# ComputationalRobotics/XM-code

Measured on AMD Instinct MI355X. Metric: BM iters/sec (tCG Hessian-vector iterations per second; ms_per_step = wall-clock-to-KKT of one staircase solve), higher is better.
Workload: dtype f64

## Files before the change

### xm-code_amd/csrc/xm_common.h

```cpp
#pragma once

#include <hip/hip_runtime.h>

#include <algorithm>
#include <cstdint>
#include <cstdio>
#include <stdexcept>
#include <string>
#include <vector>

namespace xm {

struct Error : std::runtime_error {
    int code;
    Error(int c, const std::string &m) : std::runtime_error(m), code(c) {}
};

#define XM_HIP_CHECK(expr)                                                                            \
    do {                                                                                              \
        hipError_t _e = (expr);                                                                       \
        if (_e != hipSuccess)                                                                         \
            throw ::xm::Error(-3, std::string("HIP error: ") + hipGetErrorString(_e) + " at " +       \
                                      __FILE__ + ":" + std::to_string(__LINE__) + " (" #expr ")");    \
    } while (0)
// ... 156 lines not shown
    const double *ps_cur;
    double *ps_next;
    double *vR, *vs, *HvR, *Hvs, *rR;
    const double *rs_cur;
    double *rs_next;
    double *Wloc, *Wpad;
    PointPtrs cur, cand;
    const double *partsA;
    double *partsM;
    int nM;
    double delta_bar, gradtol;
    int max_outer;
    double *trace;
    int trace_cap;
    const int *stop_req;
    unsigned long long *hprog;
    unsigned int run;
    int slot, grp;
};
void launch_outer_step(int o, int polar, const OuterStepArgs &A, int grid, hipStream_t st);

struct TcgParity {
    TcgScal *scal_cur, *scal_next;
    double *ps_cur, *ps_next, *rs_cur, *rs_next;
    size_t chunk, b_off;
    double *pcur;
    double *parts;
    double *Bout;
    double *partsB_out;
};

struct TcgInitArgs {
    int nloc;
    const double *rgR, *rgs, *R, *s;
    double *rR, *rs, *pR, *ps, *vR, *vs, *HvR, *Hvs;
    double *Wloc, *Wpad;
    TcgScal *scal0;
    double rr, delta;
    unsigned long long *hstat;
    int seq;
    const SpecCtl *spec;
};
struct CgStepArgs {
    int nloc;
    TcgParity v;
    int nA, nB, world;
    const double *HpR, *Hps, *R, *s;
    double *pR, *vR, *vs, *HvR, *Hvs, *rR;
    double *Wloc, *Wpad;
    unsigned long long *hstat;
    int64_t mat;
    double *Afull, *Wfull;
    int grouping;
    PeerXchg xchg;
};

void launch_qw_dense(int o, int epi, const double *Q, int64_t ld, const double *W, double alpha, const CamArgs &a,
                     hipStream_t st);
void launch_qw_bsr3(int o, int epi, const int64_t *rowptr, const int32_t *colidx, const double *blocks, const double *W,
                    double alpha, const CamArgs &a, hipStream_t st, int64_t nb = 0, const int4 *rowinfo = nullptr);
int64_t sell_resident_bytes(int64_t stream, int64_t other);
void bsr_build_rowinfo(const int64_t *rowptr_host, int nloc, std::vector<int4> &out);
int qw_grid(int nloc);
void launch_qw_dense_split(int o, int epi, const double *Q, int64_t ld, const double *W, double alpha, const CamArgs &a, hipStream_t st);
int qw_dense_tile_cols();
int qw_dense_split_k(int nloc, int64_t ld);
int bsr_grid(int nloc);
void qw_bench_nt(int nt);
void symv_bench_k(int k, int kf);
int symv_trace_slots();
struct SymvPlan { int K, Kf, ysplit, nchunks, gx, gy; };
void symv_plan_get(int nloc, int64_t ld, int out[4]);
struct SymvWork {
    int nloc = 0, o = 0;
    int64_t ld = 0;
    SymvPlan plan{};
    DevBuf<double> prow, pcol;
    void ensure(int nloc, int64_t ld, int o);
    void release();
    explicit operator bool() const { return pcol.p != nullptr; }
};
void launch_qw_sym_traced(int o, const double *Q, int64_t ld, const double *W, const CamArgs &a, SymvWork &work, unsigned long long *trace, hipStream_t st);
void launch_qw_sym(int o, int epi, const double *Q, int64_t ld, const double *W, double alpha, const CamArgs &a, SymvWork &work, hipStream_t st,
                   int rev = 0);
void launch_asym(const double *Q, int64_t ld, int64_t m, double *out, int grid, hipStream_t st);
void launch_dense_to_f32(const double *src, float *dst, int64_t rows, int64_t ld, unsigned int *bad, hipStream_t st);
void launch_qw_dense_f32(int o, int epi, const float *Qf, const double *Qd, int64_t ld, const double *W, double alpha, const CamArgs &a, hipStream_t st);
void launch_qw_sym_f32(int o, int epi, const float *Qf, const double *Qd, int64_t ld, const double *W, double alpha, const CamArgs &a, SymvWork &work,
                       hipStream_t st, int rev = 0);

void launch_symhash(const double *Q, int64_t ld, int64_t row0, int64_t nrows, int64_t m, unsigned long long *out, int grid, hipStream_t st);

void launch_transpose_pad(const double *src_colmajor, int64_t lds, int64_t rows, int64_t cols, double *dst, int64_t ldd,
                          hipStream_t st);
void launch_dense_from_bsr(const int64_t *rowptr, const int32_t *colidx, const double *blocks, int64_t nloc, int64_t cam0,
                           double *dst, int64_t ldd, hipStream_t st);

int flat_grid(int64_t elems);
void launch_scale_rows(int o, int nloc, const double *R, const double *s, double *Wloc, hipStream_t st);
void launch_tcg_init(int o, const TcgInitArgs &a, hipStream_t st);
void launch_cg_step(int o, const CgStepArgs &a, hipStream_t st);
struct OuterArgs { double loss, delta, delta_bar, gradtol; int shrink_count, last_iter; };
void launch_outer_finalize(const double *partsA, int nA_loc, int world, const double *partsM, int nM, const TcgScal *scal, double *hres,
                           unsigned long long seq, int grouping, hipStream_t st, const OuterArgs *oa = nullptr, SpecCtl *spec_out = nullptr);
void launch_retract(int o, int nloc, int cam0, const double *R, const double *s, const double *D, const double *ds, double t,
                    double *Rout, double *sout, double *Wloc, hipStream_t st, int polar = 0);
int retract_grid(int nloc);
void launch_retract_model(int o, int nloc, int cam0, const double *R, const double *s, const double *vR, const double *vs, double *Rout, double *sout,
                          double *Wloc, double *Wpad, const double *HvR, const double *Hvs, const double *rgR, const double *rgs, double *parts,
                          hipStream_t st, int polar);
void launch_cert_prepare(int o, int nloc, int cam0, double lam, const double *QsR, const double *R, const double *s,
                         double *Lam, double *dz, double *parts, hipStream_t st);
void launch_recover_gram(int64_t n, int r, const double *R, const double *s, double *parts, int grid, hipStream_t st);
void launch_recover_project(int64_t n, int r, const double *R, const double *s, const double *V, double *rot, double *scale, int *negcount,
                            hipStream_t st, int variant = 0);
void launch_negate(double *x, int64_t len, hipStream_t st);
int dots_multi_segments(int64_t len);
void launch_dots_multi(const double *V, int64_t ldv, int m, const double *w, int64_t len, double *c, double *scratch, hipStream_t st);
void launch_sub_vc(double *w, const double *V, int64_t ldv, const double *c, int m, int64_t len, hipStream_t st);
void launch_scale_copy(double *dst, const double *src, double a, int64_t len, hipStream_t st);
void launch_copy_words(void *dst, const void *src, size_t bytes, hipStream_t st);
void launch_lz_alpha(const double *c1j, const double *c2j, double *alpha_j, hipStream_t st);
void launch_dots_multi_parts(const double *V, int64_t ldv, int m, const double *w, int64_t len, double *scratch, hipStream_t st);
bool lz_fused_ok(int m);
void launch_sub_vc_fin(double *w, const double *V, int64_t ldv, const double *parts, int m, int64_t len, double *c_out, const double *c_prev,
                       double *alpha_j, hipStream_t st);
void launch_lz_next_fin(double *dst, const double *w, const double *parts, double *beta_j, int64_t len, hipStream_t st);
void launch_lz_next(double *dst, const double *w, const double *ww, double *beta_j, int64_t len, hipStream_t st);
void launch_gemv_n(double *y, const double *V, int64_t ldv, const double *c, int m, int64_t len, hipStream_t st);


void launch_edge_locate(int64_t ne, const int32_t *ei, const int32_t *ej, int cam0, int nloc, const int64_t *rowptr, const int32_t *colidx,
                        int64_t *pos_ij, int64_t *pos_ji, int64_t *pos_d, hipStream_t st);
void launch_edge_write(bool dense, int64_t ne, const int32_t *ei, const int32_t *ej, const double *M, const double *w, int cam0, int nloc,
                       const int64_t *inc_ptr, const int32_t *inc_edge, const int64_t *pos_ij, const int64_t *pos_ji, const int64_t *pos_d,
                       double *blocks, double *Q, int64_t ld, hipStream_t st);
void launch_edge_residual(int64_t ne, const int32_t *ei, const int32_t *ej, const double *M, const double *Y, int o, int OP, double *res,
                          hipStream_t st);

void launch_xm2_error(int64_t n, const double *w, const double *res, double *err, hipStream_t st);
void launch_radix_hist(int64_t n, const double *x, int shift, unsigned long long prefix, unsigned int *hist, hipStream_t st);
void launch_xm2_filter(int64_t n, const double *err, const double *w, double thr, double *wout, unsigned int *removed, hipStream_t st);

#define XM_DISPATCH_O(o, CALL)                                                         \
    switch (o) {                                                                       \
        case 1: { constexpr int O_ = 1; CALL; } break;                                 \
        case 3: { constexpr int O_ = 3; CALL; } break;                                 \
        case 4: { constexpr int O_ = 4; CALL; } break;                                 \
        case 5: { constexpr int O_ = 5; CALL; } break;                                 \
        case 6: { constexpr int O_ = 6; CALL; } break;                                 \
        case 7: { constexpr int O_ = 7; CALL; } break;                                 \
        case 8: { constexpr int O_ = 8; CALL; } break;                                 \
        case 9: { constexpr int O_ = 9; CALL; } break;                                 \
        case 10: { constexpr int O_ = 10; CALL; } break;                               \
        default: throw Error(-2, "rank o must be 1 or 3..10, got " + std::to_string(o)); \
    }

inline void check_launch(const char *what) {
    hipError_t e = hipGetLastError();
    if (e != hipSuccess) throw Error(-3, std::string("kernel launch failed (") + what + "): " + hipGetErrorString(e));
}

}
```

### xm-code_amd/csrc/xm_kernels.hip

```cpp
#include <algorithm>
#include <cmath>
#include <cstdlib>
#include <cstring>
#include <type_traits>

#include "xm_common.h"
#include "xm_device.h"
#include "xm_symv_step.h"

namespace xm {

__device__ __forceinline__ double2 nt_load16(const double2 *p) {
    typedef double d2v __attribute__((ext_vector_type(2)));
    const d2v v = __builtin_nontemporal_load(reinterpret_cast<const d2v *>(p));
    return make_double2(v.x, v.y);
}

template <int O, int EPI, int NSUB, bool SPLIT = false>
__global__ __launch_bounds__(256) void qw_dense_kernel(const double *__restrict__ Q, int64_t ld,
                                                        const double *__restrict__ W, double alpha, CamArgs a) {
    constexpr int OP = pitch_of(O);
    int role = EPI;
    constexpr int TILE = NSUB * 128;
    constexpr int TILE2 = TILE * OP / 2;
// ... 2068 lines not shown
        hipLaunchKernelGGL((qw_dense_kernel<1, EPI_CERT, 2>), dim3(qw_grid(a.nloc)), dim3(256), 0, st, Q, ld, W, alpha, ac);
    } else {
        XM_DISPATCH_O(o, (qw_dense_epi<O_, kQwNsub>(epi, Q, ld, W, alpha, a, st)));
    }
    check_launch("qw_dense");
}

static int64_t symv_live_groups(int64_t nsteps, int64_t nstrips, int64_t k) {
    int64_t live = 0;
    for (int64_t s = 0; s < nstrips; ++s) live += (std::min<int64_t>(nsteps, (s * kSvStrip + kSvStrip + 5) / 6) + 4 * k - 1) / (4 * k);
    return live;
}
int symv_k(int nloc, int64_t ld) {
    const int64_t nsteps = (nloc + 1) / 2, nstrips = (ld + kSvStrip - 1) / kSvStrip;
    int64_t total = 0;
    for (int64_t s = 0; s < nstrips; ++s) total += std::min<int64_t>(nsteps, (s * kSvStrip + kSvStrip + 5) / 6);
    int64_t k = (int64_t)(std::sqrt((double)total) / 18.0 + 0.5);
    k = std::min<int64_t>(64, std::max<int64_t>(2, k));
    if (symv_live_groups(nsteps, nstrips, k) <= 1100) {
        int64_t ks = 4;
        while (symv_live_groups(nsteps, nstrips, ks) > 504) ++ks;
        k = ks;
    }
    return (int)k;
}
static int g_symv_k = 0, g_symv_kf = 0;
void symv_bench_k(int k, int kf) { g_symv_k = k; g_symv_kf = kf; }
static SymvPlan symv_plan(int nloc, int64_t ld) {
    SymvPlan p;
    p.K = g_symv_k > 0 ? g_symv_k : symv_k(nloc, ld);
    const int nsteps = (nloc + 1) / 2, nstrips = (int)((ld + kSvStrip - 1) / kSvStrip);
    p.gy = (nstrips + 1) / 2;
    if (g_symv_k > 0 && g_symv_kf > 0) {
        p.Kf = std::min(g_symv_kf, p.K);
        p.ysplit = (int)(0.75 * p.gy);
    } else if (p.K >= 8 && symv_live_groups(nsteps, nstrips, p.K) > 1100) {
        p.Kf = p.K / 4;
        p.ysplit = (int)(0.75 * p.gy);
    } else {
        p.Kf = p.K; p.ysplit = p.gy;
    }
    auto groups = [&](int s, int k) { return (int)((std::min<int64_t>(nsteps, ((int64_t)s * kSvStrip + kSvStrip + 5) / 6) + 4 * k - 1) / (4 * k)); };
    p.gx = 1;
    for (int y = 0; y < p.gy; ++y) {
        const int k = (y >= p.ysplit) ? p.Kf : p.K, sb = nstrips - 1 - y;
        p.gx = std::max(p.gx, groups(y, k) + (sb != y ? groups(sb, k) : 0));
    }
    p.nchunks = (nsteps + 4 * p.Kf - 1) / (4 * p.Kf);
    return p;
}
void symv_plan_get(int nloc, int64_t ld, int out[4]) {
    const SymvPlan p = symv_plan(nloc, ld);
    out[0] = p.K; out[1] = p.Kf; out[2] = p.ysplit; out[3] = p.nchunks;
}
void SymvWork::ensure(int nloc_new, int64_t ld_new, int o_new) {
    release();
    const SymvPlan p = symv_plan(nloc_new, ld_new);
    prow.alloc((size_t)((ld_new + kSvStrip - 1) / kSvStrip) * 6 * (size_t)((nloc_new + 1) / 2) * o_new);
    pcol.alloc((size_t)p.nchunks * (size_t)ld_new * o_new, false);
    nloc = nloc_new; ld = ld_new; o = o_new; plan = p;
}
void SymvWork::release() {
    prow.release(); pcol.release();
    nloc = 0; ld = 0; o = 0; plan = SymvPlan{};
}
struct SymvGeom { dim3 gs; int rK, rKf, ys, nstrips; };
static SymvGeom symv_geom(const SymvWork &w, int nloc, int64_t ld, int o) {
    if (!w || nloc != w.nloc || ld != w.ld || o > w.o) throw Error(-2, "symmetric product: the workspace was not made for this size and rank");
    return {dim3(w.plan.gx, w.plan.gy), 4 * w.plan.K, 4 * w.plan.Kf, w.plan.ysplit, (int)((ld + kSvStrip - 1) / kSvStrip)};
}

static int symv_nt_step0(int nloc, double elem_bytes) {
    const double m = 3.0 * nloc;
    const double tri = elem_bytes * m * (m + 6.0) / 2.0;
    const int64_t res = qw_resident_bytes((size_t)tri);
    const int nsteps = (nloc + 1) / 2;
    if ((double)res >= tri) return nsteps + 1;
    const double disc = m * m - 2.0 * (double)res / elem_bytes;
    const double r = m - std::sqrt(std::max(0.0, disc));
    return (int)std::min<double>(nsteps + 1, std::max(0.0, r / 6.0));
}
template <int O>
static void qw_symv_epi(int epi, const double *Q, int64_t ld, const double *W, double alpha, const CamArgs &a, SymvWork &work,
                        hipStream_t st, int rev, unsigned long long *trace = nullptr) {
    const auto [gs, rK, rKf, ys, nstrips] = symv_geom(work, a.nloc, ld, O);
    const SymvPlan &pl = work.plan;
    double *const Prow = work.prow.p, *const Pcol = work.pcol.p;
    const TcgScal *sc = (epi == EPI_HESS || epi == EPI_AUTO) ? a.scal : (const TcgScal *)nullptr;
    const int by_phase = (epi == EPI_AUTO) ? 1 : 0;
    const int nt0 = symv_nt_step0(a.nloc, sizeof(double));
    if (trace) {
        if constexpr (O == 3 || O == 4) hipLaunchKernelGGL((qw_symv_kernel<O, true>), gs, dim3(256), 0, st, Q, ld, W, a.nloc, pl.K, pl.Kf, ys, nt0, sc, Prow, Pcol, trace, rev, by_phase);
    } else hipLaunchKernelGGL((qw_symv_kernel<O>), gs, dim3(256), 0, st, Q, ld, W, a.nloc, pl.K, pl.Kf, ys, nt0, sc, Prow, Pcol, trace, rev, by_phase);
    const dim3 g(qw_grid(a.nloc)), b(256);
    switch (epi) {
        case EPI_PLAIN: hipLaunchKernelGGL((symv_reduce_kernel<O, EPI_PLAIN>), g, b, 0, st, Prow, Pcol, ld, nstrips, rK, rKf, ys, alpha, a); break;
        case EPI_GRAD: hipLaunchKernelGGL((symv_reduce_kernel<O, EPI_GRAD>), g, b, 0, st, Prow, Pcol, ld, nstrips, rK, rKf, ys, alpha, a); break;
        case EPI_HESS: hipLaunchKernelGGL((symv_reduce_kernel<O, EPI_HESS>), g, b, 0, st, Prow, Pcol, ld, nstrips, rK, rKf, ys, alpha, a); break;
        case EPI_AUTO:
            if constexpr (O >= 3) { hipLaunchKernelGGL((symv_reduce_kernel<O, EPI_AUTO>), g, b, 0, st, Prow, Pcol, ld, nstrips, rK, rKf, ys, alpha, a); break; }
            throw Error(-2, "bad epilogue");
        case EPI_CERT:
            if constexpr (O == 1) { hipLaunchKernelGGL((symv_reduce_kernel<1, EPI_CERT>), g, b, 0, st, Prow, Pcol, ld, nstrips, rK, rKf, ys, alpha, a); break; }
            throw Error(-2, "certificate operator needs o == 1");
        default: throw Error(-2, "bad epilogue");
    }
}
int symv_trace_slots() { return kSvTraceSlots; }
void launch_qw_sym_traced(int o, const double *Q, int64_t ld, const double *W, const CamArgs &a, SymvWork &work, unsigned long long *trace, hipStream_t st) {
    if (trace == nullptr) throw Error(-2, "traced symmetric product: no trace buffer");
    if (o == 3) qw_symv_epi<3>(EPI_PLAIN, Q, ld, W, 1.0, a, work, st, 0, trace);
    else if (o == 4) qw_symv_epi<4>(EPI_PLAIN, Q, ld, W, 1.0, a, work, st, 0, trace);
    else throw Error(-2, "traced symmetric product: o = 3 or 4");
    check_launch("qw_symv traced");
}

void launch_qw_sym(int o, int epi, const double *Q, int64_t ld, const double *W, double alpha, const CamArgs &a, SymvWork &work, hipStream_t st,
                   int rev) {
    if (a.nloc <= 0) return;
    switch (o) {
        case 1: qw_symv_epi<1>(epi, Q, ld, W, alpha, a, work, st, rev & 1); break;
        case 3: qw_symv_epi<3>(epi, Q, ld, W, alpha, a, work, st, rev & 1); break;
        case 4: qw_symv_epi<4>(epi, Q, ld, W, alpha, a, work, st, rev & 1); break;
        case 5: qw_symv_epi<5>(epi, Q, ld, W, alpha, a, work, st, rev & 1); break;
        default: throw Error(-2, "symmetric product is instantiated for o = 1, 3..5");
    }
    check_launch("qw_symv");
}
__global__ __launch_bounds__(256) void symhash_kernel(const double *__restrict__ Q, int64_t ld, int64_t row0, int64_t nrows, int64_t m,
                                                       unsigned long long *out) {
    __shared__ unsigned long long sh[2][4];
    unsigned long long acc = 0ull, bad = 0ull;
    const int64_t total = nrows * m;
    for (int64_t e = (int64_t)blockIdx.x * 256 + threadIdx.x; e < total; e += (int64_t)gridDim.x * 256) {
        const int64_t lr = e / m, c = e - lr * m, r = row0 + lr;
        if (r >= m || r == c) continue;
        const double v = Q[lr * ld + c];
        if (v != v) bad = 1ull;
        unsigned long long b = (v == 0.0) ? 0ull : (unsigned long long)__double_as_longlong(v);
        unsigned long long z = (unsigned long long)((r < c) ? r : c) * 0x9E3779B97F4A7C15ull + (unsigned long long)((r < c) ? c : r);
        z = (z ^ (z >> 30)) * 0xBF58476D1CE4E5B9ull; z = (z ^ (z >> 27)) * 0x94D049BB133111EBull; z ^= z >> 31;
        const unsigned long long t = (z | 1ull) * b;
        acc += (r < c) ? t : (0ull - t);
    }
    for (int off = 32; off > 0; off >>= 1) { acc += __shfl_xor(acc, off, 64); bad |= __shfl_xor(bad, off, 64); }
    if ((threadIdx.x & 63) == 0) { sh[0][threadIdx.x >> 6] = acc; sh[1][threadIdx.x >> 6] = bad; }
    __syncthreads();
    if (threadIdx.x == 0) {
        out[2 * blockIdx.x] = sh[0][0] + sh[0][1] + sh[0][2] + sh[0][3];
        out[2 * blockIdx.x + 1] = sh[1][0] | sh[1][1] | sh[1][2] | sh[1][3];
    }
}
void launch_symhash(const double *Q, int64_t ld, int64_t row0, int64_t nrows, int64_t m, unsigned long long *out, int grid, hipStream_t st) {
    hipLaunchKernelGGL(symhash_kernel, dim3(grid), dim3(256), 0, st, Q, ld, row0, nrows, m, out);
    check_launch("symhash");
}
void launch_asym(const double *Q, int64_t ld, int64_t m, double *out, int grid, hipStream_t st) {
    hipLaunchKernelGGL(asym_kernel, dim3(grid), dim3(256), 0, st, Q, ld, m, out);
    check_launch("asym");
}

template <int O, int VAR>
static void qw_bsr3_epi(int epi, const int64_t *rp, const int32_t *ci, const double *bl, const double *W, const int4 *ri, double alpha,
                        const CamArgs &a, hipStream_t st) {
    const dim3 g((a.nloc + kBsrRows - 1) / kBsrRows), b(256);
    switch (epi) {
        case EPI_PLAIN: hipLaunchKernelGGL((qw_bsr3_kernel<O, EPI_PLAIN, VAR>), g, b, 0, st, rp, ci, bl, W, ri, alpha, a); break;
        case EPI_GRAD: hipLaunchKernelGGL((qw_bsr3_kernel<O, EPI_GRAD, VAR>), g, b, 0, st, rp, ci, bl, W, ri, alpha, a); break;
        case EPI_HESS: hipLaunchKernelGGL((qw_bsr3_kernel<O, EPI_HESS, VAR>), g, b, 0, st, rp, ci, bl, W, ri, alpha, a); break;
        case EPI_AUTO:
            if constexpr (O >= 3) { hipLaunchKernelGGL((qw_bsr3_kernel<O, EPI_AUTO, VAR>), g, b, 0, st, rp, ci, bl, W, ri, alpha, a); break; }
            throw Error(-2, "bad epilogue");
        default: throw Error(-2, "bad epilogue");
    }
}
static int bsr_nt_cam0(int nloc, int64_t nb) {
    const size_t bytes = (size_t)std::max<int64_t>(nb, 0) * 76;
    return qw_resident_bytes(bytes) >= (int64_t)bytes ? nloc : 0;
}
void bsr_build_rowinfo(const int64_t *rowptr_host, int nloc, std::vector<int4> &out) {
    out.resize((size_t)std::max(nloc, 0));
    for (int c0 = 0; c0 < nloc; c0 += kBsrRows) {
        const int m = std::min(kBsrRows, nloc - c0);
        int order[kBsrRows];
        for (int j = 0; j < m; ++j) order[j] = c0 + j;
        std::stable_sort(order, order + m, [&](int x, int y) {
            return (rowptr_host[x + 1] - rowptr_host[x] + 15) / 16 > (rowptr_host[y + 1] - rowptr_host[y] + 15) / 16;
        });
        for (int j = 0; j < m; ++j) {
            const int i = order[j];
            const int64_t b0 = rowptr_host[i], len = rowptr_host[i + 1] - b0;
            if (len >= ((int64_t)1 << 31)) throw Error(-2, "block-CSR row with 2^31 or more blocks");
            out[(size_t)c0 + j] = make_int4((int)(unsigned)(b0 & 0xffffffffll), (int)(unsigned)((unsigned long long)b0 >> 32), (int)len, i);
        }
    }
}
void launch_qw_bsr3(int o, int epi, const int64_t *rp, const int32_t *ci, const double *bl, const double *W, double alpha,
                    const CamArgs &a0, hipStream_t st, int64_t nb, const int4 *ri) {
    if (a0.nloc <= 0) return;
    CamArgs a = a0;
    a.nt_cam0 = bsr_nt_cam0(a.nloc, nb);
    if (epi == EPI_CERT) {
        if (o != 1) throw Error(-2, "certificate operator needs o == 1");
        hipLaunchKernelGGL((qw_bsr3_kernel<1, EPI_CERT, 0>), dim3((a.nloc + kBsrRows - 1) / kBsrRows), dim3(256), 0, st, rp, ci, bl, W, ri, alpha, a);
    } else {
        switch (o) {
            case 3: qw_bsr3_epi<3, 2>(epi, rp, ci, bl, W, ri, alpha, a, st); break;
// ... 506 lines not shown
```

### xm-code_amd/csrc/xm_solver.h

```cpp
#pragma once

#include <chrono>
#include <cstdint>
#include <cstdio>
#include <memory>
#include <string>
#include <vector>

#include "../../include/xm_amd.h"
#include "xm_common.h"

namespace xm {

struct Settings {
    int sym = 0;
    int64_t sym_min_rows = 0;
    int64_t sym_rows(int world) const { return sym_min_rows > 0 ? sym_min_rows : (world <= 1 ? 4096 : 6144); }
    int sell = 0;
    int sell_slabs = 4, sell_lmax = 64, sell_gather = 1;
    int sell_codec = 0;
    int sell_wpad = 0;
    int overlap = 0;
    double overlap_min_mb = 64.0;
    int64_t cert_dense_rows = 384;
// ... 134 lines not shown
    DevBuf<double> Afull_;
    DevBuf<int64_t> rowptr_;
    DevBuf<int32_t> colidx_;
    DevBuf<double> blocks_;
    int64_t nb_loc_ = 0;
    DevBuf<int4> rowinfo_;
    std::unique_ptr<SellMatrix> sell_;
    int sell_gm_ = 0;
    std::unique_ptr<SchurOp> schur_;
    bool schur_dense_ = false;
    int64_t ne_ = 0;
    DevBuf<int32_t> ei_, ej_, inc_edge_;
    DevBuf<int64_t> inc_ptr_, pos_ij_, pos_ji_, pos_d_;
    DevBuf<double> eM_, ew_, eres_;
    bool solved_ = false;
    std::vector<double> w_cur_;
    DevBuf<double> eerr_;
    const double *residuals_recovered_device(const double *rot, const double *scale);
    hipStream_t st_ = nullptr;
    hipStream_t st2_ = nullptr;
    hipEvent_t ev_w_ = nullptr, ev_p_ = nullptr;
    DevBuf<double> Pstrip_;
    bool w_pending_ = false;
    std::shared_ptr<Comm> comm_;
    Settings cfg_;
    PeerXchg xchg_;
    double *partsB_peer_ = nullptr;
    unsigned long long tcg_runs_ = 0;
    std::vector<int64_t> cam_cut_;
    int retraction_ = 0, grouping_ = 0;

    int o_ = 0, OP_ = 0;
    DevBuf<double> R_, s_, Rc_, sc_, W_, D_;
    DevBuf<double> wpad_;
    double *wpad() const { return (wpad_.p && wpad_on_) ? wpad_.p : nullptr; }
    bool wpad_on_ = false;
    const double *wpad_next_ = nullptr;
    PointState ps_[2];
    int cur_ = 0;
    DevBuf<double> rR_, rs_, rsB_, pR_, psA_, psB_, vR_, vs_, HvR_, Hvs_, HpR_, Hps_;
    DevBuf<double> partsA_, partsB_, partsM_;
    SymvWork symv_;
    DevBuf<double> ksum_;
    DevBuf<unsigned int> kcount_;
    int ks_ = 1;
    std::unique_ptr<SymwProduct> symw_;
    void product_symw(int epi, int o, double alpha, const CamArgs &a);
    bool sym_ok_ = false;
    int sym_max_o_ = 4;
    bool eig_exact_ = false;
    double q_asym_ = 0, q_max_ = 0;
    DevBuf<TcgScal> scal_;
    unsigned long long *hstat_ = nullptr;
    unsigned long long *hstat_dev_ = nullptr;
    double *hpin_ = nullptr;
    double *hpin_dev_ = nullptr;
    size_t hpin_count_ = 0;
    int nA_ = 0, nB_ = 0;
    unsigned long long outer_seq_ = 0;

    const xm_options_t *opt_ = nullptr;
    xm_result_t *res_ = nullptr;
    bool verbose_ = false;
    std::vector<std::pair<hipEvent_t, hipEvent_t>> ev_pool_;
    size_t ev_used_ = 0;
    int64_t hess_launches_ = 0;
    int sym_rev_ = 1;
    std::vector<float> qw_samples_;

    void init(const xm_problem_t &prob);
    void to_host(void *dst, const void *src_dev, size_t bytes);
    void to_dev(void *dst_dev, const void *src, size_t bytes);
    void ensure_pinned(size_t doubles);
    DevBuf<double> lzV_, lzc_, lzw_, lzc2_, lzab_, lzscr_;
    DevBuf<double> recW_;
    int64_t pos_of(int64_t g) const;
    void release_raw();
    void setup_rank(int o);
    void upload_point(const std::vector<double> &R_cm, int o, const std::vector<double> &s_ex);
    void download_point(std::vector<double> &R_cm, std::vector<double> &s_ex);
    CamArgs cam_args(int state) const;
    int prod_grid() const;
    int tcg_blocks() const;
    void product(int epi, int o, double alpha, const CamArgs &a);
    void gather_W();
    void flush_gather();
    bool overlap_applies() const;
    void eval_point(int state, const double *Rp, const double *sp, double &f, double &rr);
    double sum_parts(const double *dparts, int count);
    int run_tcg(double rr, double delta, int adopted = 0);
    int enqueue_spec_tcg();
    void tcg_enqueue_iteration(int i, bool profile);
    TcgParity tcg_parity(int par) const;
    void cand_role(CamArgs &a, const PointState &P, const double *R, const double *s) const;
    CamArgs tcg_cam_args(const TcgParity &v, bool cand) const;
    void tcg_product(int epi, const CamArgs &a, int par, bool profile);
    TcgInitArgs tcg_init_args(double rr, double delta, const SpecCtl *spec) const;
    CgStepArgs cg_step_args(int i) const;
    void probe_grad(bool aut, double &f, double &rr);
    bool spec_applies() const;
    DevBuf<SpecCtl> spec_;
    unsigned int tcg_seq_ = 0;
    volatile double *wait_outer_result();
    bool stream_idle(std::chrono::steady_clock::time_point t_wait, const char *what);
    bool agree_any(bool local);
    void drain_events();
    void finish_profile();
    TrResult trust_region(int o, double &gradtol, double linesearch_step, const std::vector<double> &v_dir, double max_time);
    bool device_outer_applies(int o) const;
    TrResult trust_region_device(int o, double &gradtol, double f, double rr, double delta, double delta_bar, double max_time);
    OuterStepArgs outer_step_args(int slot, bool model_rec, double delta_bar, double gradtol, unsigned int runid) const;
    void progress_line(int k, int inner, double loss, double gradnorm, int endreason, int trstatus) const;
    TrResult close_trust_region(int stop_reason, double &gradtol, long long totalite, int k, double loss, std::chrono::steady_clock::time_point start);
    DevBuf<double> trace_dev_;
    DevBuf<int> stop_req_;
    DevBuf<OuterScal> oscal_;
    unsigned int outer_run_ = 0;
    CertResult certificate(int o, double primal, std::vector<double> &v_out);
    int cert_multipliers(int o, double lam);
    int lanczos_min(std::vector<double> &x_out, double &theta, int &iters, double &resid);
    int lz_m_use_ = 0, lz_cycles_ = 0;
    bool lz_unfused_ = false;
    void cert_product(const double *vj, const CamArgs &a, int j);
    void log(const char *fmt, ...) const;
};

void tridiag_min_export(const double *a, const double *b, int m, double *theta, double *y, double *tmax);

class Team {
public:
    Team(const xm_problem_t &prob, int n_gpus, int gpu_map);
    ~Team();
    Team(const Team &) = delete;
    Team &operator=(const Team &) = delete;
    int world() const;
    int comm_kind() const;
    int product_kind(int o) const;
    const std::string &fallback_note() const;
    void solve(const xm_options_t &opt, xm_result_t &res);
    void attach_edges(int64_t ne, const int32_t *ei, const int32_t *ej, const double *M);
    void edge_residuals(double *res);
    void set_edge_weights(const double *w);
    void edge_residuals_recovered(const double *rot, const double *scale, double *res);
    double xm2_filter(const double *rot, const double *scale, double pct, int64_t *removed, double *w_out);
    int64_t cameras() const;
    std::vector<double> weights() const;
private:
    struct Impl;
    std::unique_ptr<Impl> p_;
    void shutdown();
};

}
```

### xm-code_amd/csrc/xm_solver.hip

```cpp
#include "xm_solver.h"
#include "xm_sell.h"
#include "xm_symw.h"
#include "xm_schur.h"
#include "xm_ba.h"
#include "xm_clean.h"
#include "xm_trackfilter.h"

#include <algorithm>
#include <chrono>
#include <cmath>
#include <cstdarg>
#include <cstdlib>
#include <cstring>
#include <thread>

namespace xm {

using clk = std::chrono::steady_clock;
static double secs_since(clk::time_point t0) { return std::chrono::duration<double>(clk::now() - t0).count(); }

void Context::log(const char *fmt, ...) const {
    if (!verbose_ || (comm_ && comm_->rank != 0)) return;
    va_list ap;
    va_start(ap, fmt);
// ... 448 lines not shown
        kcount_.alloc((size_t)qw_grid(nloc_));
    }
    if (overlap_applies()) {
        if (!st2_) {
            XM_HIP_CHECK(hipStreamCreateWithFlags(&st2_, hipStreamNonBlocking));
            XM_HIP_CHECK(hipEventCreateWithFlags(&ev_w_, hipEventDisableTiming));
            XM_HIP_CHECK(hipEventCreateWithFlags(&ev_p_, hipEventDisableTiming));
        }
        Pstrip_.alloc(mat);
    }
    scal_.ensure(2, st_);
    spec_.ensure(1, st_);
    if (sell_ && sell_supports(o)) (void)sell_->parts(o);
    ensure_pinned(std::max<size_t>((size_t)2 * nA_ + (size_t)nB_ + partsM_.count + 64, (size_t)ld_ * OP_ + (size_t)ntot_ + 1024));
    if (comm_->active()) comm_->host_barrier();
}

void Context::upload_point(const std::vector<double> &R_cm, int o, const std::vector<double> &s_ex) {
    const size_t m = (size_t)3 * n_;
    std::vector<double> Rr((size_t)nloc_ * 3 * OP_, 0.0), sl((size_t)nloc_, 1.0);
    for (int c = 0; c < nloc_; ++c) {
        const bool real = c < true_loc_;
        const int64_t g = g0_ + c;
        for (int a = 0; a < 3; ++a)
            for (int k = 0; k < o; ++k)
                Rr[((size_t)c * 3 + a) * OP_ + k] = real ? R_cm[(size_t)(3 * g + a) + (size_t)k * m] : (a == k ? 1.0 : 0.0);
        if (real) sl[(size_t)c] = s_ex[(size_t)g];
    }
    if (cam0_ == 0) sl[0] = 1.0;
    to_dev(R_.p, Rr.data(), Rr.size() * sizeof(double));
    to_dev(s_.p, sl.data(), sl.size() * sizeof(double));
}

void Context::download_point(std::vector<double> &R_cm, std::vector<double> &s_ex) {
    const size_t m = (size_t)3 * n_, mat = (size_t)nloc_ * 3 * OP_;
    std::vector<double> full((size_t)ntot_ * 3 * OP_), sf((size_t)ntot_);
    launch_scale_copy(W_.p + (size_t)comm_->rank * mat, R_.p, 1.0, (int64_t)mat, st_);
    if (comm_->active()) comm_->allgather(W_.p, mat, st_);
    to_host(full.data(), W_.p, full.size() * sizeof(double));
    launch_scale_copy(W_.p + (size_t)comm_->rank * nloc_, s_.p, 1.0, (int64_t)nloc_, st_);
    if (comm_->active()) comm_->allgather(W_.p, (size_t)nloc_, st_);
    to_host(sf.data(), W_.p, sf.size() * sizeof(double));
    XM_HIP_CHECK(hipMemsetAsync(W_.p, 0, W_.count * sizeof(double), st_));
    R_cm.assign(m * (size_t)o_, 0.0);
    s_ex.assign((size_t)n_, 1.0);
    for (int64_t g = 0; g < n_; ++g) {
        const size_t q = (size_t)pos_of(g);
        for (int a = 0; a < 3; ++a)
            for (int k = 0; k < o_; ++k) R_cm[(size_t)(3 * g + a) + (size_t)k * m] = full[(q * 3 + a) * OP_ + k];
        s_ex[(size_t)g] = sf[q];
    }
}

int Context::prod_grid() const {
    if (storage_ == XM_STORAGE_BSR3 && sell_ && sell_supports(o_)) return sell_->reduce_grid(o_, nloc_);
    return (storage_ == XM_STORAGE_BSR3) ? bsr_grid(nloc_) : qw_grid(nloc_);
}

int Context::tcg_blocks() const {
    int g = flat_grid((int64_t)nloc_ * 3 * OP_);
    if (comm_->peer() && comm_->world > 1 && cfg_.exchange != 1 && !symw_ && storage_ != XM_STORAGE_SCHUR && comm_->device_waits()) g = std::min(g, std::max(8, 1024 / std::max(1, comm_->ranks_on_my_device())));
    return g;
}

CamArgs Context::cam_args(int state) const {
    CamArgs a;
    std::memset(&a, 0, sizeof(a));
    a.nloc = nloc_;
    a.cam0 = cam0_;
    a.lam = opt_ ? opt_->lam : 0.0;
    a.R = R_.p;
    a.s = s_.p;
    const PointState &p = ps_[state];
    a.G = p.G.p; a.egs = p.egs.p; a.S0 = p.S0.p; a.rgR = p.rgR.p; a.rgs = p.rgs.p;
    a.pR = pR_.p; a.ps = psA_.p; a.rR = rR_.p; a.rs = rs_.p; a.HpR = HpR_.p; a.Hps = Hps_.p;
    a.Wloc = W_.p + (size_t)cam0_ * 3 * OP_;
    a.out = HpR_.p;
    a.partials = partsA_.p;
    a.scal = scal_.p;
    if (ks_ > 1) { a.ks = ks_; a.ksum = ksum_.p; a.kcount = kcount_.p; }
    return a;
}

void Context::product(int epi, int o, double alpha, const CamArgs &a) {
    if (w_pending_) {
        if (storage_ == XM_STORAGE_DENSE && (epi == EPI_PLAIN || epi == EPI_GRAD) && o == o_) {
            w_pending_ = false;
            const int tc = qw_dense_tile_cols();
            const int64_t c0 = 3 * (int64_t)cam0_, c1 = 3 * ((int64_t)cam0_ + nloc_);
            CamArgs s1 = a, s2 = a;
            s1.range_mode = 1; s1.t_lo = (int)((c0 + tc - 1) / tc); s1.t_hi = (int)(c1 / tc); s1.out = Pstrip_.p; s1.addend = nullptr;
            s2.range_mode = 2; s2.t_lo = s1.t_lo; s2.t_hi = s1.t_hi; s2.addend = Pstrip_.p;
            comm_->note("overlap_split", (double)s1.t_lo, (double)s1.t_hi);
            XM_HIP_CHECK(hipEventRecord(ev_w_, st_));
            XM_HIP_CHECK(hipStreamWaitEvent(st2_, ev_w_, 0));
            launch_qw_dense_split(o, EPI_PLAIN, dQ_, ld_, W_.p, 1.0, s1, st2_);
            XM_HIP_CHECK(hipEventRecord(ev_p_, st2_));
            comm_->allgather(W_.p, (size_t)nloc_ * 3 * OP_, st_);
            XM_HIP_CHECK(hipStreamWaitEvent(st_, ev_p_, 0));
            launch_qw_dense_split(o, epi, dQ_, ld_, W_.p, alpha, s2, st_);
            if (res_) res_->qw_products++;
            return;
        }
        flush_gather();
    }
    if (storage_ == XM_STORAGE_DENSE && dQ32_ && o == o_ && (epi == EPI_HESS || epi == EPI_AUTO)) {
        if (sym_ok_ && o >= 3 && o <= sym_max_o_ && symv_) launch_qw_sym_f32(o, epi, dQ32_, dQ_, ld_, W_.p, alpha, a, symv_, st_, sym_rev_);
        else { CamArgs ar = a; ar.rev = sym_rev_; launch_qw_dense_f32(o, epi, dQ32_, dQ_, ld_, W_.p, alpha, ar, st_); }
    } else if (storage_ == XM_STORAGE_DENSE) {
        if (symw_ && o == o_ && o >= 3 && o <= sym_max_o_ && epi != EPI_CERT) product_symw(epi, o, alpha, a);
        else if (sym_ok_ && o == o_ && o >= 3 && o <= sym_max_o_ && epi != EPI_CERT && symv_) launch_qw_sym(o, epi, dQ_, ld_, W_.p, alpha, a, symv_, st_, sym_rev_);
        else { CamArgs ar = a; ar.rev = sym_rev_; launch_qw_dense(o, epi, dQ_, ld_, W_.p, alpha, ar, st_); }
    } else if (storage_ == XM_STORAGE_SCHUR) {
        schur_->product(o, epi, W_.p, alpha, a, st_);
    } else if (sell_ && sell_supports(o)) {
        const double *wp = (epi == EPI_HESS && o == o_) ? wpad() : ((epi == EPI_GRAD && o == o_) ? wpad_next_ : nullptr);
        wpad_next_ = nullptr;
        launch_qw_sell(o, epi, *sell_, W_.p, alpha, a, sell_gm_, st_, wp);
    } else {
        launch_qw_bsr3(o, epi, rowptr_.p, colidx_.p, blocks_.p, W_.p, alpha, a, st_, nb_loc_, rowinfo_.p);
    }
    if (res_) res_->qw_products++;
}

int Context::product_kind(int o) const {
    if (storage_ == XM_STORAGE_SCHUR) return XM_PRODUCT_SCHUR;
    if (storage_ == XM_STORAGE_DENSE) return ((symw_ || sym_ok_) && o >= 3 && o <= sym_max_o_) ? XM_PRODUCT_DENSE_SYM : XM_PRODUCT_DENSE;
    if (sell_ && sell_supports(o)) return sell_->codec() == SELL_CODEC_QUAT ? XM_PRODUCT_SELL_QUAT : XM_PRODUCT_SELL;
    return XM_PRODUCT_BSR3;
}

void Context::product_symw(int epi, int o, double alpha, const CamArgs &a) {
    symw_->sweep(o, dQ_, W_.p, (epi == EPI_HESS) ? a.scal : (const TcgScal *)nullptr, comm_->rank, st_);
    comm_->allgather(symw_->csum_all(), symw_->csum_count(o), st_);
    symw_->reduce(o, epi, alpha, a, comm_->world, st_);
}

bool Context::overlap_applies() const {
    if (cfg_.overlap < 0 || !comm_->active() || storage_ != XM_STORAGE_DENSE || sym_ok_ || symw_) return false;
    if ((double)nloc_ * 3.0 * (double)ld_ * 8.0 < cfg_.overlap_min_mb * 1048576.0) return false;
    const int tc = qw_dense_tile_cols();
    const int64_t c0 = 3 * (int64_t)cam0_, c1 = 3 * ((int64_t)cam0_ + nloc_);
    return (c1 / tc) > ((c0 + tc - 1) / tc);
}

void Context::gather_W() {
    if (!comm_->active()) return;
    if (overlap_applies()) { w_pending_ = true; return; }
    comm_->allgather(W_.p, (size_t)nloc_ * 3 * OP_, st_);
}

void Context::flush_gather() {
    if (!w_pending_) return;
    w_pending_ = false;
    comm_->allgather(W_.p, (size_t)nloc_ * 3 * OP_, st_);
}

double Context::sum_parts(const double *dparts, int count) {
    if (comm_->peer()) launch_copy_words(hpin_dev_, dparts, (size_t)count * sizeof(double), st_);
    else XM_HIP_CHECK(hipMemcpyAsync(hpin_, dparts, (size_t)count * sizeof(double), hipMemcpyDeviceToHost, st_));
    XM_HIP_CHECK(hipStreamSynchronize(st_));
    double t = 0.0;
    for (int i = 0; i < count; ++i) t += hpin_[i];
    return t;
}

void Context::eval_point(int state, const double *Rp, const double *sp, double &f, double &rr) {
    const int nA_loc = prod_grid();
    CamArgs a = cam_args(state);
    a.R = Rp;
    a.s = sp;
    a.partials = partsA_.p + (size_t)comm_->rank * 2 * nA_loc;
    product(EPI_GRAD, o_, 2.0, a);
    if (comm_->active()) comm_->allgather(partsA_.p, (size_t)2 * nA_loc, st_);
    launch_outer_finalize(partsA_.p, nA_loc, comm_->world, partsM_.p, 0, scal_.p, reinterpret_cast<double *>(hstat_dev_) + 8,
                          ++outer_seq_, grouping_, st_);
    volatile double *hres = wait_outer_result();
    f = hres[0];
    rr = hres[1];
}

bool Context::agree_any(bool local) {
    if (!comm_->active()) return local;
    const int world = comm_->world;
    double v = local ? 1.0 : 0.0;
    to_dev(partsM_.p + comm_->rank, &v, sizeof(double));
    comm_->allgather(partsM_.p, 1, st_);
    if (comm_->peer()) launch_copy_words(hpin_dev_, partsM_.p, (size_t)world * sizeof(double), st_);
    else XM_HIP_CHECK(hipMemcpyAsync(hpin_, partsM_.p, (size_t)world * sizeof(double), hipMemcpyDeviceToHost, st_));
    XM_HIP_CHECK(hipStreamSynchronize(st_));
    bool any = false;
    for (int r = 0; r < world; ++r) any = any || (hpin_[r] != 0.0);
    return any;
}

bool Context::stream_idle(clk::time_point t_wait, const char *what) {
    const double limit = cfg_.watchdog_s;
    comm_->check_device_error();
    const hipError_t q = hipStreamQuery(st_);
    if (q == hipSuccess) return true;
    if (q != hipErrorNotReady) {
        (void)hipGetLastError();
        throw Error(XM_ERR_HIP, std::string("device error while waiting for ") + what + ": " + hipGetErrorString(q));
    }
    if (secs_since(t_wait) > limit)
        throw Error(XM_ERR_HIP, std::string("watchdog: no progress for ") + std::to_string((int)limit) + " s while waiting for " + what);
    return false;
}

volatile double *Context::wait_outer_result() {
    volatile unsigned long long *hseq = reinterpret_cast<volatile unsigned long long *>(hstat_) + 8 + 5;
    const unsigned long long seq = outer_seq_;
    const auto t_wait = clk::now();
    auto t_check = t_wait;
    while (*hseq != seq) {
        __builtin_ia32_pause();
        if (secs_since(t_check) > 500e-6) {
            if (stream_idle(t_wait, "the outer-iteration results")) {
                XM_HIP_CHECK(hipStreamSynchronize(st_));
                if (*hseq != seq) throw Error(XM_ERR_HIP, "outer-iteration results did not reach host-mapped memory");
            }
            t_check = clk::now();
        }
    }
    return reinterpret_cast<volatile double *>(hstat_) + 8;
}

void Context::drain_events() {
    for (size_t i = 0; i < ev_used_; ++i) {
        float ms = 0.f;
        if (hipEventElapsedTime(&ms, ev_pool_[i].first, ev_pool_[i].second) == hipSuccess) qw_samples_.push_back(ms);
    }
    ev_used_ = 0;
}

void Context::finish_profile() {
    drain_events();
    if (qw_samples_.empty()) return;
    std::vector<float> v = qw_samples_;
    std::sort(v.begin(), v.end());
    const float ref = v[(v.size() * 3) / 4];
    for (float x : v)
        if (x >= 0.5f * ref) { res_->qw_ms_sum += x; res_->qw_ms_count++; }
    qw_samples_.clear();
}

void Context::tcg_enqueue_iteration(int i, bool profile) {
    const CgStepArgs S = cg_step_args(i);
    tcg_product(EPI_HESS, tcg_cam_args(S.v, false), i & 1, profile);
    if (comm_->active() && xchg_.world <= 1) comm_->allgather(S.v.pcur, S.v.chunk, st_);
    launch_cg_step(o_, S, st_);
}

TcgParity Context::tcg_parity(int par) const {
    const size_t nA = (size_t)prod_grid(), world = (size_t)comm_->world, rank = (size_t)comm_->rank;
    TcgParity v;
    v.scal_cur = scal_.p + par; v.scal_next = scal_.p + (par ^ 1);
    v.ps_cur = par ? psB_.p : psA_.p; v.ps_next = par ? psA_.p : psB_.p;
    v.rs_cur = par ? rsB_.p : rs_.p; v.rs_next = par ? rs_.p : rsB_.p;
    v.b_off = comm_->active() ? (size_t)nloc_ * 3 * OP_ : 0;
    v.chunk = v.b_off + 3 * nA + (size_t)tcg_blocks();
    double *pB = xchg_.world > 1 ? partsB_peer_ : partsB_.p;
    v.pcur = pB + (size_t)par * v.chunk * world;
    v.parts = v.pcur + rank * v.chunk + v.b_off;
    v.Bout = comm_->active() ? v.pcur + rank * v.chunk : nullptr;
    v.partsB_out = pB + (size_t)(par ^ 1) * v.chunk * world + rank * v.chunk + v.b_off + 3 * nA;
    return v;
}

void Context::cand_role(CamArgs &a, const PointState &P, const double *R, const double *s) const {
    a.cand = {R, s, P.G.p, P.egs.p, P.S0.p, P.rgR.p, P.rgs.p, partsA_.p};
}

CamArgs Context::tcg_cam_args(const TcgParity &v, bool cand) const {
    CamArgs a = cam_args(cur_);
    a.scal = v.scal_cur; a.ps = v.ps_cur; a.rs = v.rs_cur;
    a.partials = v.parts; a.Bout = v.Bout;
    if (cand) cand_role(a, ps_[cur_ ^ 1], Rc_.p, sc_.p);
    return a;
}

void Context::tcg_product(int epi, const CamArgs &a, int par, bool profile) {
    const bool timed = profile && (hess_launches_ % kProfileStride == 0) && ev_used_ < ev_pool_.size();
    if (timed) XM_HIP_CHECK(hipEventRecord(ev_pool_[ev_used_].first, st_));
    sym_rev_ = par;
    product(epi, o_, 2.0, a);
    sym_rev_ = 1;
    if (timed) { XM_HIP_CHECK(hipEventRecord(ev_pool_[ev_used_].second, st_)); ev_used_++; }
    hess_launches_++;
}

TcgInitArgs Context::tcg_init_args(double rr, double delta, const SpecCtl *spec) const {
    const PointState &P = ps_[cur_];
    TcgInitArgs a;
    a.nloc = nloc_;
    a.rgR = P.rgR.p; a.rgs = P.rgs.p; a.R = R_.p; a.s = s_.p;
    a.rR = rR_.p; a.rs = rs_.p; a.pR = pR_.p; a.ps = psA_.p; a.vR = vR_.p; a.vs = vs_.p; a.HvR = HvR_.p; a.Hvs = Hvs_.p;
    a.Wloc = wpad() ? nullptr : W_.p + (size_t)cam0_ * 3 * OP_; a.Wpad = wpad();
    a.scal0 = scal_.p; a.rr = rr; a.delta = delta;
    a.hstat = hstat_dev_; a.seq = (int)tcg_seq_; a.spec = spec;
    return a;
}

CgStepArgs Context::cg_step_args(int i) const {
    const bool model_rec = opt_ && (opt_->flags & XM_FLAG_MODEL_RECURRENCE);
    CgStepArgs a;
    a.nloc = nloc_; a.v = tcg_parity(i & 1);
    a.nA = prod_grid(); a.nB = tcg_blocks(); a.world = comm_->world;
    a.HpR = HpR_.p; a.Hps = Hps_.p; a.R = R_.p; a.s = s_.p;
    a.pR = pR_.p; a.vR = vR_.p; a.vs = vs_.p; a.HvR = model_rec ? nullptr : HvR_.p; a.Hvs = model_rec ? nullptr : Hvs_.p; a.rR = rR_.p;
    a.Wloc = wpad() ? nullptr : W_.p + (size_t)cam0_ * 3 * OP_; a.Wpad = wpad();
    a.hstat = hstat_dev_; a.mat = (int64_t)nloc_ * 3 * OP_;
    a.Afull = comm_->active() ? Afull_.p : nullptr; a.Wfull = W_.p;
    a.grouping = grouping_; a.xchg = xchg_;
    return a;
}

bool Context::spec_applies() const {
    return !comm_->active() && opt_ && !(opt_->flags & XM_FLAG_HOST_STEPPED) && storage_ != XM_STORAGE_SCHUR && cfg_.debug_drop_finalize < 0;
}

int Context::enqueue_spec_tcg() {
    std::swap(R_.p, Rc_.p);
    std::swap(s_.p, sc_.p);
    cur_ ^= 1;
    ++tcg_seq_;
    launch_tcg_init(o_, tcg_init_args(0.0, 0.0, spec_.p), st_);
    const int n_spec = 1;
    for (int i = 0; i < n_spec; ++i) tcg_enqueue_iteration(i, false);
    std::swap(R_.p, Rc_.p);
    std::swap(s_.p, sc_.p);
    cur_ ^= 1;
    return n_spec;
}

int Context::run_tcg(double rr, double delta, int adopted) {
    const bool stepped = (opt_->flags & XM_FLAG_HOST_STEPPED) != 0;
    const bool profile = (opt_->flags & XM_FLAG_PROFILE_QW) != 0;
    if (comm_->active()) comm_->note("tcg_start", rr, delta);
    if (adopted == 0) {
        ++tcg_seq_;
        launch_tcg_init(o_, tcg_init_args(rr, delta, nullptr), st_);
        gather_W();
    }
    const bool fused = xchg_.world > 1;
    if (fused) xchg_.epoch_base = (++tcg_runs_) << 12;
    const bool lockstep = comm_->active() && !fused;
    const int run_ahead = (lockstep || prod_grid() >= 64) ? 2 : 3;
    int fin_status = 0, fin_iter = 0;
    int it = adopted;
    auto enqueue = [&](int i) { tcg_enqueue_iteration(i, profile); };
    auto read_scal = [&](int par) {
        TcgScal sc;
        to_host(&sc, scal_.p + par, sizeof(TcgScal));
        return sc;
    };
    if (stepped) {
        for (;;) {
            TcgScal sc = read_scal(it & 1);
            if (sc.status != 0 || it >= kMaxInner) break;
            enqueue(it++);
        }
    } else {
        volatile unsigned long long *hs = hstat_;
        auto last_progress = clk::now();
        auto last_change = last_progress;
        unsigned long long seen = ~0ull;
        for (;;) {
            const unsigned long long v = *hs;
            if (v != seen) { seen = v; last_progress = clk::now(); last_change = last_progress; }
            const bool valid = (unsigned int)(v >> 32) == tcg_seq_;
            const int status = valid ? (int)(v & 0xff) : 0;
            const int done = valid ? (int)((v >> 8) & 0xffffff) : 0;
            if (status != 0) { fin_status = status; fin_iter = done; break; }
            if (it < kMaxInner && it - done < run_ahead) { enqueue(it++); continue; }
            __builtin_ia32_pause();
            if (secs_since(last_progress) > 200e-6) {
                if (stream_idle(last_change, "the truncated-CG progress word")) {
                    TcgScal sc = read_scal(it & 1);
                    if (sc.status != 0) { fin_status = sc.status; fin_iter = sc.iter; break; }
                    if (it >= kMaxInner) { fin_status = 6; fin_iter = kMaxInner; break; }
                    *hstat_ = ((unsigned long long)tcg_seq_ << 32) | ((unsigned long long)(unsigned)sc.iter << 8);
                    if (it - sc.iter >= run_ahead) enqueue(it++);
                }
                last_progress = clk::now();
            }
        }
    }
    if (comm_->active()) comm_->note("tcg_end_before_topup", (double)it, (double)(fin_iter * 16 + fin_status));
    if (fin_status == 7) { comm_->check_device_error(); throw Error(XM_ERR_COMM, "peer exchange: a rank did not arrive inside the truncated CG"); }
    if (lockstep && !stepped) {
        const int T = (fin_status == 6) ? fin_iter - 1 : fin_iter;
        while (it < std::min(kMaxInner, T + 2)) enqueue(it++);
    }
    return it;
}

TrResult Context::trust_region(int o, double &gradtol, double linesearch_step, const std::vector<double> &v_dir, double max_time) {
    TrResult out;
    const double dim = (double)n_ * (3.0 * o - 6.0) + (double)n_ - 1.0;
    const double delta_bar = std::sqrt(dim);
    double delta = delta_bar / 8.0;
    double *Wloc = W_.p + (size_t)cam0_ * 3 * OP_;
    double f = 0, rr = 0;

    log("start linesearch\n");
    if (linesearch_step != 0) {
        launch_scale_rows(o, nloc_, R_.p, s_.p, Wloc, st_);
        gather_W();
        double f0, tmp;
        eval_point(cur_ ^ 1, R_.p, s_.p, f0, tmp);
        double alpha = linesearch_step;
        std::vector<double> D((size_t)nloc_ * 3 * OP_, 0.0);
        for (int c = 0; c < (int)true_loc_; ++c) {
            const int64_t g = g0_ + c;
            for (int a = 0; a < 3; ++a) D[((size_t)c * 3 + a) * OP_ + (o - 1)] = v_dir[(size_t)(3 * g + a)];
        }
        to_dev(D_.p, D.data(), D.size() * sizeof(double));
        double fn;
        for (;;) {
            launch_retract(o, nloc_, cam0_, R_.p, s_.p, D_.p, nullptr, -alpha, Rc_.p, nullptr, Wloc, st_, retraction_);
            gather_W();
            eval_point(cur_ ^ 1, Rc_.p, s_.p, fn, tmp);
            if (!(fn > f0)) break;
            alpha *= 0.5;
            if (alpha < 1e-20) { log("linesearch failed! BM stopped! \n"); out.primal = -1; out.ls_failed = true; out.stop_reason = -1; return out; }
        }
        if (f0 - fn > 0) {
            log("linesearch decrease %1.3e\n", f0 - fn);
            if (opt_->flags & XM_FLAG_FIX_STALE_SR) {
                std::swap(R_.p, Rc_.p);
                launch_scale_rows(o, nloc_, R_.p, s_.p, Wloc, st_);
            } else {
                launch_scale_rows(o, nloc_, R_.p, s_.p, Wloc, st_);
                std::swap(R_.p, Rc_.p);
            }
            gather_W();
        } else {
            log("linesearch failed! BM stopped! \n");
            out.primal = -1; out.ls_failed = true; out.stop_reason = -1;
            return out;
        }
    } else {
        launch_scale_rows(o, nloc_, R_.p, s_.p, Wloc, st_);
        gather_W();
    }
    eval_point(cur_, R_.p, s_.p, f, rr);
    if (device_outer_applies(o)) return trust_region_device(o, gradtol, f, rr, delta, delta_bar, max_time);
    double loss = f;

    int endreason = 6, trstatus = 4, shrink_count = 0, inner_print = 1, k = 0;
    int adopted = 0;
    long long totalite = 0;
    int stop_reason = 14;
    const auto start = clk::now();
    for (k = 0; k < kMaxOuter; ++k) {
        const double gradnorm = std::sqrt(rr);
        progress_line(k, inner_print, loss, gradnorm, endreason, trstatus);
        if (opt_->trace && res_->trace_len < opt_->trace_cap) {
            double *tr = opt_->trace + (size_t)res_->trace_len * 6;
            tr[0] = loss; tr[1] = gradnorm; tr[2] = inner_print; tr[3] = endreason; tr[4] = trstatus; tr[5] = delta;
            res_->trace_len++;
        }
        if (endreason == 5) { stop_reason = 5; break; }
        if (gradnorm < gradtol) { stop_reason = 10; break; }
        if (agree_any((double)(long long)secs_since(start) > max_time)) { stop_reason = 11; break; }
        endreason = 6; trstatus = 4;

        TcgScal fin;
        const int enq = run_tcg(rr, delta, adopted);
        adopted = 0;
// ... 1371 lines not shown
```

Before: 24310.

## Split tCG Hessian product into head/tail phases for tighter host enqueue

Splits the symmetric Hessian-vector product into a head phase (the main symv kernel) and a tail phase (the reduce kernel plus the CG step). The host loop now enqueues these separately, gated on device progress, instead of queueing whole iterations up to a run-ahead depth. The aim is to keep the next product's heavy kernel queued while less speculative work is submitted past the termination point. The risk is that lower run-ahead exposes host launch latency and gaps between kernels. It also adds bookkeeping for profiling events and product counts.

New measurement: 24240. Within noise of the previous version (-0.3%).

```diff
diff --git a/xm-code_amd/csrc/xm_common.h b/xm-code_amd/csrc/xm_common.h
--- a/xm-code_amd/csrc/xm_common.h
+++ b/xm-code_amd/csrc/xm_common.h
@@ -262,7 +262,7 @@
 };
 void launch_qw_sym_traced(int o, const double *Q, int64_t ld, const double *W, const CamArgs &a, SymvWork &work, unsigned long long *trace, hipStream_t st);
 void launch_qw_sym(int o, int epi, const double *Q, int64_t ld, const double *W, double alpha, const CamArgs &a, SymvWork &work, hipStream_t st,
-                   int rev = 0);
+                   int rev = 0, int phase = 0);
 void launch_asym(const double *Q, int64_t ld, int64_t m, double *out, int grid, hipStream_t st);
 void launch_dense_to_f32(const double *src, float *dst, int64_t rows, int64_t ld, unsigned int *bad, hipStream_t st);
 void launch_qw_dense_f32(int o, int epi, const float *Qf, const double *Qd, int64_t ld, const double *W, double alpha, const CamArgs &a, hipStream_t st);
diff --git a/xm-code_amd/csrc/xm_kernels.hip b/xm-code_amd/csrc/xm_kernels.hip
--- a/xm-code_amd/csrc/xm_kernels.hip
+++ b/xm-code_amd/csrc/xm_kernels.hip
@@ -2174,16 +2174,18 @@
 }
 template <int O>
 static void qw_symv_epi(int epi, const double *Q, int64_t ld, const double *W, double alpha, const CamArgs &a, SymvWork &work,
-                        hipStream_t st, int rev, unsigned long long *trace = nullptr) {
+                        hipStream_t st, int rev, unsigned long long *trace = nullptr, int phase = 0) {
     const auto [gs, rK, rKf, ys, nstrips] = symv_geom(work, a.nloc, ld, O);
     const SymvPlan &pl = work.plan;
     double *const Prow = work.prow.p, *const Pcol = work.pcol.p;
     const TcgScal *sc = (epi == EPI_HESS || epi == EPI_AUTO) ? a.scal : (const TcgScal *)nullptr;
     const int by_phase = (epi == EPI_AUTO) ? 1 : 0;
     const int nt0 = symv_nt_step0(a.nloc, sizeof(double));
-    if (trace) {
+    if (phase == 2) {
+    } else if (trace) {
         if constexpr (O == 3 || O == 4) hipLaunchKernelGGL((qw_symv_kernel<O, true>), gs, dim3(256), 0, st, Q, ld, W, a.nloc, pl.K, pl.Kf, ys, nt0, sc, Prow, Pcol, trace, rev, by_phase);
     } else hipLaunchKernelGGL((qw_symv_kernel<O>), gs, dim3(256), 0, st, Q, ld, W, a.nloc, pl.K, pl.Kf, ys, nt0, sc, Prow, Pcol, trace, rev, by_phase);
+    if (phase == 1) return;
     const dim3 g(qw_grid(a.nloc)), b(256);
     switch (epi) {
         case EPI_PLAIN: hipLaunchKernelGGL((symv_reduce_kernel<O, EPI_PLAIN>), g, b, 0, st, Prow, Pcol, ld, nstrips, rK, rKf, ys, alpha, a); break;
@@ -2208,13 +2210,13 @@
 }
 
 void launch_qw_sym(int o, int epi, const double *Q, int64_t ld, const double *W, double alpha, const CamArgs &a, SymvWork &work, hipStream_t st,
-                   int rev) {
+                   int rev, int phase) {
     if (a.nloc <= 0) return;
     switch (o) {
-        case 1: qw_symv_epi<1>(epi, Q, ld, W, alpha, a, work, st, rev & 1); break;
-        case 3: qw_symv_epi<3>(epi, Q, ld, W, alpha, a, work, st, rev & 1); break;
-        case 4: qw_symv_epi<4>(epi, Q, ld, W, alpha, a, work, st, rev & 1); break;
-        case 5: qw_symv_epi<5>(epi, Q, ld, W, alpha, a, work, st, rev & 1); break;
+        case 1: qw_symv_epi<1>(epi, Q, ld, W, alpha, a, work, st, rev & 1, nullptr, phase); break;
+        case 3: qw_symv_epi<3>(epi, Q, ld, W, alpha, a, work, st, rev & 1, nullptr, phase); break;
+        case 4: qw_symv_epi<4>(epi, Q, ld, W, alpha, a, work, st, rev & 1, nullptr, phase); break;
+        case 5: qw_symv_epi<5>(epi, Q, ld, W, alpha, a, work, st, rev & 1, nullptr, phase); break;
         default: throw Error(-2, "symmetric product is instantiated for o = 1, 3..5");
     }
     check_launch("qw_symv");
diff --git a/xm-code_amd/csrc/xm_solver.h b/xm-code_amd/csrc/xm_solver.h
--- a/xm-code_amd/csrc/xm_solver.h
+++ b/xm-code_amd/csrc/xm_solver.h
@@ -240,7 +240,7 @@
     CamArgs cam_args(int state) const;
     int prod_grid() const;
     int tcg_blocks() const;
-    void product(int epi, int o, double alpha, const CamArgs &a);
+    void product(int epi, int o, double alpha, const CamArgs &a, int phase = 0);
     void gather_W();
     void flush_gather();
     bool overlap_applies() const;
@@ -249,10 +249,15 @@
     int run_tcg(double rr, double delta, int adopted = 0);
     int enqueue_spec_tcg();
     void tcg_enqueue_iteration(int i, bool profile);
+    void tcg_enqueue_head(int i, bool profile);
+    void tcg_enqueue_tail(int i);
+    bool tcg_pair() const;
+    bool tcg_rotates() const;
+    bool head_timed_ = false;
     TcgParity tcg_parity(int par) const;
     void cand_role(CamArgs &a, const PointState &P, const double *R, const double *s) const;
     CamArgs tcg_cam_args(const TcgParity &v, bool cand) const;
-    void tcg_product(int epi, const CamArgs &a, int par, bool profile);
+    void tcg_product(int epi, const CamArgs &a, int par, bool profile, int phase = 0);
     TcgInitArgs tcg_init_args(double rr, double delta, const SpecCtl *spec) const;
     CgStepArgs cg_step_args(int i) const;
     void probe_grad(bool aut, double &f, double &rr);
diff --git a/xm-code_amd/csrc/xm_solver.hip b/xm-code_amd/csrc/xm_solver.hip
--- a/xm-code_amd/csrc/xm_solver.hip
+++ b/xm-code_amd/csrc/xm_solver.hip
@@ -554,7 +554,7 @@
     return a;
 }
 
-void Context::product(int epi, int o, double alpha, const CamArgs &a) {
+void Context::product(int epi, int o, double alpha, const CamArgs &a, int phase) {
     if (w_pending_) {
         if (storage_ == XM_STORAGE_DENSE && (epi == EPI_PLAIN || epi == EPI_GRAD) && o == o_) {
             w_pending_ = false;
@@ -581,8 +581,10 @@
         else { CamArgs ar = a; ar.rev = sym_rev_; launch_qw_dense_f32(o, epi, dQ32_, dQ_, ld_, W_.p, alpha, ar, st_); }
     } else if (storage_ == XM_STORAGE_DENSE) {
         if (symw_ && o == o_ && o >= 3 && o <= sym_max_o_ && epi != EPI_CERT) product_symw(epi, o, alpha, a);
-        else if (sym_ok_ && o == o_ && o >= 3 && o <= sym_max_o_ && epi != EPI_CERT && symv_) launch_qw_sym(o, epi, dQ_, ld_, W_.p, alpha, a, symv_, st_, sym_rev_);
-        else { CamArgs ar = a; ar.rev = sym_rev_; launch_qw_dense(o, epi, dQ_, ld_, W_.p, alpha, ar, st_); }
+        else if (sym_ok_ && o == o_ && o >= 3 && o <= sym_max_o_ && epi != EPI_CERT && symv_) {
+            launch_qw_sym(o, epi, dQ_, ld_, W_.p, alpha, a, symv_, st_, sym_rev_, phase);
+            if (phase == 1) return;
+        } else { CamArgs ar = a; ar.rev = sym_rev_; launch_qw_dense(o, epi, dQ_, ld_, W_.p, alpha, ar, st_); }
     } else if (storage_ == XM_STORAGE_SCHUR) {
         schur_->product(o, epi, W_.p, alpha, a, st_);
     } else if (sell_ && sell_supports(o)) {
@@ -722,6 +724,21 @@
     tcg_product(EPI_HESS, tcg_cam_args(S.v, false), i & 1, profile);
     if (comm_->active() && xchg_.world <= 1) comm_->allgather(S.v.pcur, S.v.chunk, st_);
     launch_cg_step(o_, S, st_);
+}
+
+void Context::tcg_enqueue_head(int i, bool profile) {
+    tcg_product(EPI_HESS, tcg_cam_args(tcg_parity(i & 1), false), i & 1, profile, 1);
+}
+void Context::tcg_enqueue_tail(int i) {
+    const CgStepArgs S = cg_step_args(i);
+    tcg_product(EPI_HESS, tcg_cam_args(S.v, false), i & 1, false, 2);
+    launch_cg_step(o_, S, st_);
+}
+bool Context::tcg_pair() const {
+    return storage_ == XM_STORAGE_DENSE && !dQ32_ && !symw_ && sym_ok_ && o_ >= 3 && o_ <= sym_max_o_ && symv_;
+}
+bool Context::tcg_rotates() const {
+    return !comm_->active() && opt_ && !(opt_->flags & XM_FLAG_HOST_STEPPED) && storage_ == XM_STORAGE_DENSE && !dQ32_ && !symw_ && ks_ <= 1;
 }
 
 TcgParity Context::tcg_parity(int par) const {
@@ -752,14 +769,18 @@
     return a;
 }
 
-void Context::tcg_product(int epi, const CamArgs &a, int par, bool profile) {
-    const bool timed = profile && (hess_launches_ % kProfileStride == 0) && ev_used_ < ev_pool_.size();
-    if (timed) XM_HIP_CHECK(hipEventRecord(ev_pool_[ev_used_].first, st_));
+void Context::tcg_product(int epi, const CamArgs &a, int par, bool profile, int phase) {
+    const bool split = phase != 0 && tcg_pair();
+    if (phase == 2 && !split) return;
+    const bool timed = (phase == 2) ? head_timed_ : (profile && (hess_launches_ % kProfileStride == 0) && ev_used_ < ev_pool_.size());
+    if (timed && phase != 2) XM_HIP_CHECK(hipEventRecord(ev_pool_[ev_used_].first, st_));
     sym_rev_ = par;
-    product(epi, o_, 2.0, a);
+    product(epi, o_, 2.0, a, split ? phase : 0);
     sym_rev_ = 1;
+    if (split && phase == 1) { head_timed_ = timed; hess_launches_++; return; }
     if (timed) { XM_HIP_CHECK(hipEventRecord(ev_pool_[ev_used_].second, st_)); ev_used_++; }
-    hess_launches_++;
+    head_timed_ = false;
+    if (phase != 2) hess_launches_++;
 }
 
 TcgInitArgs Context::tcg_init_args(double rr, double delta, const SpecCtl *spec) const {
@@ -821,6 +842,8 @@
     const int run_ahead = (lockstep || prod_grid() >= 64) ? 2 : 3;
     int fin_status = 0, fin_iter = 0;
     int it = adopted;
+    const bool rotate = tcg_rotates();
+    int heads = adopted;
     auto enqueue = [&](int i) { tcg_enqueue_iteration(i, profile); };
     auto read_scal = [&](int par) {
         TcgScal sc;
@@ -845,7 +868,10 @@
             const int status = valid ? (int)(v & 0xff) : 0;
             const int done = valid ? (int)((v >> 8) & 0xffffff) : 0;
             if (status != 0) { fin_status = status; fin_iter = done; break; }
-            if (it < kMaxInner && it - done < run_ahead) { enqueue(it++); continue; }
+            if (rotate) {
+                if (it < heads && it <= done) { tcg_enqueue_tail(it++); continue; }
+                if (heads == it && heads < kMaxInner && heads <= done + 1) { tcg_enqueue_head(heads++, profile); continue; }
+            } else if (it < kMaxInner && it - done < run_ahead) { enqueue(it++); continue; }
             __builtin_ia32_pause();
             if (secs_since(last_progress) > 200e-6) {
                 if (stream_idle(last_change, "the truncated-CG progress word")) {
@@ -853,12 +879,13 @@
                     if (sc.status != 0) { fin_status = sc.status; fin_iter = sc.iter; break; }
                     if (it >= kMaxInner) { fin_status = 6; fin_iter = kMaxInner; break; }
                     *hstat_ = ((unsigned long long)tcg_seq_ << 32) | ((unsigned long long)(unsigned)sc.iter << 8);
-                    if (it - sc.iter >= run_ahead) enqueue(it++);
+                    if (!rotate && it - sc.iter >= run_ahead) enqueue(it++);
                 }
                 last_progress = clk::now();
             }
         }
     }
+    if (rotate && heads > it && !tcg_pair() && res_) res_->qw_products--;
     if (comm_->active()) comm_->note("tcg_end_before_topup", (double)it, (double)(fin_iter * 16 + fin_status));
     if (fin_status == 7) { comm_->check_device_error(); throw Error(XM_ERR_COMM, "peer exchange: a rank did not arrive inside the truncated CG"); }
     if (lockstep && !stepped) {
```
